# qmoututu11/Image_Restoration_and_Enhancement

Hardware: AMD Instinct MI355X
Metric: restored images/sec @512x512, 50 DDIM steps; PSNR/SSIM vs reference (higher is better)
Workload: dtype bf16; 1 GPU; BASELINE configs[1] denoise 512x512, batch 8/GPU, 50 DDIM steps x strength 0.5 = 25 UNet evals, CFG 5.0 (UNet batch 16); task=denoise, global_batch=8, resolution=512, compute=UNet + CLIP bf16, VAE fp16 (fp32 accumulation), parallelism=dp1, weights_bcast=none, outputs_finite=True

## Files before the change

image_restoration_and_enhancement_amd/_lib.py:

```python
from __future__ import annotations

import ctypes as C
import os
from pathlib import Path

_PKG = Path(__file__).resolve().parent
LIB_PATH = Path(os.environ.get("IRX_LIB", _PKG / "libirx.so"))

IRX_F32, IRX_BF16, IRX_F16 = 0, 1, 2
IRX_MODEL_UNET, IRX_MODEL_VAE, IRX_MODEL_CLIP = 0, 1, 2
IRX_MODEL_LPIPS = 3
IRX_MODEL_FID = 4
IRX_MODEL_SRVGG = 5
IRX_LAYOUT_VEC, IRX_LAYOUT_MAT, IRX_LAYOUT_CONV, IRX_LAYOUT_EMB = 0, 1, 2, 3
IRX_LAYOUT_MAT_GEGLU64, IRX_LAYOUT_VEC_GEGLU64 = 4, 5
IRX_LAYOUT_VEC_LN_U, IRX_LAYOUT_VEC_LN_V = 6, 7
IRX_LAYOUT_MAT_CHAIN, IRX_LAYOUT_VEC_CHAIN = 8, 9
IRX_LAYOUT_CONV_UP2 = 10
IRX_RCCL_ID_BYTES = 128
IRX_RESAMPLE_LANCZOS, IRX_RESAMPLE_BICUBIC, IRX_RESAMPLE_MAX_KSIZE = 0, 1, 97


class IrxError(RuntimeError):
    pass
# ... 139 lines not shown
    "irx_op_gn_proj": (i32, [vp, i32, vp, i32, i32, i32, i32, f32, vp, vp, vp, vp, i32, vp, vp, C.POINTER(i32),
                             C.POINTER(i32)]),
    "irx_op_layer_norm": (i32, [vp, i32, vp, i32, i32, f32, vp, vp, vp]),
    "irx_op_attention": (i32, [vp, i32, i32, i32, i32, i32, i32, vp, i64, i64, vp, i64, i64, vp, i64, i64, vp,
                               i64, i64, f32, i32]),
    "irx_op_attention_hm": (i32, [vp, i32, i32, i32, i32, i32, i32, vp, vp, vp, vp, f32]),
    "irx_op_geglu": (i32, [vp, i32, vp, i32, i32, vp]),
    "irx_op_gemm_geglu": (i32, [vp, i32, i32, i32, i32, vp, vp, vp, vp]),
    "irx_op_gemm_ln_out": (i32, [vp, i32, i32, i32, i32, vp, vp, vp, vp, vp, vp, i32, f32]),
    "irx_op_gemm_ln_fold": (i32, [vp, i32, i32, i32, i32, vp, vp, vp, vp, vp, vp, i32, i32, vp]),
    "irx_op_gemm_ln_out_w": (i32, [vp, i32, i32, i32, i32, vp, vp, vp, vp, i64, vp, vp, i32, i32, f32]),
    "irx_op_gemm_ln_fold_w": (i32, [vp, i32, i32, i32, i32, vp, vp, vp, vp, vp, vp, i32, i32, i32, vp]),
    "irx_op_conv2d_gn_parts": (i32, [vp, i32, vp, vp, i32, i32, i32, i32, i32, i32, i32, vp, vp, i32, i32, i32, i32,
                                     i32, i32, i32, i32, vp, i64, vp, vp, i32, i32, vp, vp, C.POINTER(i32),
                                     C.POINTER(i32), C.POINTER(i32), C.POINTER(sz)]),
    "irx_op_gemm_gn_parts": (i32, [vp, i32, i32, i32, i32, vp, vp, vp, vp, i32, vp, vp, vp, C.POINTER(i32),
                                   C.POINTER(i32), C.POINTER(sz)]),
    "irx_op_upsample_conv_gn_parts": (i32, [vp, i32, vp, i32, i32, i32, i32, vp, vp, vp, vp, vp, C.POINTER(i32),
                                            C.POINTER(i32), C.POINTER(sz)]),
    "irx_op_group_norm_parts": (i32, [vp, i32, vp, vp, i32, i32, i32, i32, i32, f32, vp, vp, i32, vp, vp, i32, vp, i32,
                                      vp]),
    "irx_op_group_norm_parts_ab": (i32, [vp, i32, i32, i32, i32, f32, vp, vp, vp, i32, vp, vp]),
    "irx_op_softmax_rows": (i32, [vp, i32, vp, i64, i32, i32, vp, i64]),
    "irx_op_transpose2d": (i32, [vp, i32, vp, i64, i32, i32, vp, i64, i32, i64, i64]),
    "irx_op_timestep_embed": (i32, [vp, i32, vp, i32, i32, i32, f32, vp]),
    "irx_op_embed_tokens": (i32, [vp, i32, vp, i32, i32, vp, vp, i32, vp]),
}

EXPORTED = tuple(_SIGS)

_DEBUG_SIGS = {
    "irx_debug_gemm_tile": (i32, [i32, i32, i32, i32, i32, i32, C.POINTER(i32)]),
    "irx_debug_conv_plan": (i32, [i32] * 17 + [C.POINTER(i32)]),
}
_SIGS.update(_DEBUG_SIGS)

_lib = None


def load(path: Path | str | None = None, force: bool = False):
    global _lib
    if _lib is not None and not force:
        return _lib
    p = Path(path) if path else LIB_PATH
    if not p.exists():
        raise IrxError(f"native library not built: {p} (run `python -m image_restoration_and_enhancement_amd.build`)")
    lib = C.CDLL(str(p))
    for name, (res, args) in _SIGS.items():
        fn = getattr(lib, name)
        fn.restype = res
        fn.argtypes = args
    _lib = lib
    return lib


def call(name: str, *args):
    lib = load()
    rc = getattr(lib, name)(*args)
    if _SIGS[name][0] is i32 and name not in ("irx_version", "irx_rccl_available") and rc != 0:
        raise IrxError(f"{name}: {lib.irx_last_error().decode(errors='replace')}")
    return rc


def get_option(name: str) -> int:
    v = C.c_int()
    call("irx_get_option", name.encode(), C.byref(v))
# ... 50 lines not shown
```

image_restoration_and_enhancement_amd/csrc/capi.cpp:

```cpp
#include <algorithm>
#include <cmath>
#include <cstring>
#include <string>

#include "../../include/irx.h"
#include "gemm_plan.h"
#include "models.h"
#include "profile.h"

namespace irx {
static thread_local std::string g_err;
void set_error(const std::string& m) { g_err = m; }
const char* last_error() { return g_err.c_str(); }
extern int g_attn_pf80;
}

using namespace irx;

struct irx_model {
  std::unique_ptr<Model> m;
};

#define IRX_API_BEGIN try {
#define IRX_API_END                                       \
// ... 31 lines not shown

const char* irx_last_error(void) { return last_error(); }
int irx_version(void) { return 1; }

struct OptRef {
  int* i = nullptr;
  bool* b = nullptr;
};
static const struct { const char* name; int* i; bool* b; } kOpts[] = {
    {"large_tiles", nullptr, &g_large_tiles},
    {"gemm_deep", &g_gemm_deep, nullptr},
    {"gemm_dbg", &g_gemm_dbg, nullptr},
    {"gn_v2", nullptr, &g_gn_v2},
    {"gn_fuse", &g_gn_fuse, nullptr},
    {"gn_parts", &g_gn_parts, nullptr},
    {"gn_red_parts", &g_gn_red_parts, nullptr},
    {"ff_chain", &g_ff_chain, nullptr},
    {"up2", &g_up2, nullptr},
    {"ln_parts", &g_ln_parts, nullptr},
    {"gn_fold", &g_gn_fold, nullptr},
    {"gn_narrow", &g_gn_narrow, nullptr},
    {"attn_pf", &g_attn_pf, nullptr},
    {"attn_pf160", &g_attn_pf160, nullptr},
    {"attn_pf80", &g_attn_pf80, nullptr},
    {"attn_q2", &g_attn_q2, nullptr},
    {"conv1x1_dense", &g_conv1x1_dense, nullptr},
    {"gn_fa", &g_gn_fa, nullptr},
    {"gn_fa_wide", &g_gn_fa_wide, nullptr},
    {"gn_fa_blocks", &g_gn_fa_blocks, nullptr},
    {"halo_split", &g_halo_split, nullptr},
    {"halo_pipe", &g_halo_pipe, nullptr},
    {"gemm_pp", &g_gemm_pp, nullptr},
    {"gemm_pp2", &g_gemm_pp2, nullptr},
    {"ln_fold", &g_ln_fold, nullptr},
    {"gemm_sk", &g_gemm_sk, nullptr},
    {"large_mask", &g_large_mask, nullptr},
    {"large_dense", &g_large_dense, nullptr},
    {"arena_guard", &g_arena_guard, nullptr},
    {"gemm_nmajor", &g_gemm_nmajor, nullptr},
    {"halo_group", &g_halo_group, nullptr},
    {"halo_strip", &g_halo_strip, nullptr},
    {"halo_up2", &g_halo_up2, nullptr},
    {"halo_mi", &g_halo_mi, nullptr},
    {"gemm_group", &g_gemm_group, nullptr},
    {"small_splitk", &g_small_splitk, nullptr},
    {"gemm_pp_chain", &g_gemm_pp_chain, nullptr},
    {"prof_shapes", &g_prof_shapes, nullptr},
    {"attn_prio", &g_attn_prio, nullptr},
    {"attn_qrep", &g_attn_qrep, nullptr},
    {"op_imgs", &g_op_imgs, nullptr},
    {"cfg_share", &g_cfg_share, nullptr},
    {"temb_table", &g_temb_table, nullptr},
    {"gemm_sk_blocks", &g_gemm_sk_blocks, nullptr},
    {"vae_attn_rows", &g_vae_attn_rows, nullptr},
    {"vae_flash", &g_vae_flash, nullptr},
    {"splitk_inkernel", nullptr, &g_splitk_inkernel},
    {"tile_256x320", nullptr, &g_tile_256x320},
    {"gemm_force", &g_gemm_force, nullptr},
    {"conv_halo", &g_conv_halo, nullptr},
    {"gemm_small", nullptr, &g_gemm_small},
    {"attn_xcd", &g_attn_xcd, nullptr},
    {"attn_hm", &g_attn_hm, nullptr},
    {"gemm_small_kmax", &g_gemm_small_kmax, nullptr},
    {"nlm2_strip", &g_nlm2_strip, nullptr},
    {"srvgg_fused", &g_srvgg_fused, nullptr},
    {"srvgg_blocks", &g_srvgg_blocks, nullptr},
// ... 682 lines not shown
  IRX_API_END
}

size_t irx_op_gemm_workspace_bytes(int dtype, int M, int N, int K, int act, int out_f32, int imgs) {
  GemmArgs a;
  a.dtype = dtype; a.M = M; a.N = N; a.K = K;
  a.A = (const void*)(uintptr_t)4096; a.lda = K;
  a.B = (const void*)(uintptr_t)4096; a.ldb = K;
  a.C = (void*)(uintptr_t)4096; a.ldc = N;
  a.act = act; a.out_f32 = out_f32; a.imgs = imgs;
  return gemm_workspace_bytes(a);
}

int irx_debug_gemm_tile(int dtype, int M, int N, int K, int geglu, int imgs, int* tile) {
  IRX_API_BEGIN
  IRX_CHECK(tile, "null argument");
  GemmArgs a;
  a.dtype = dtype; a.M = M; a.N = N; a.K = K;
  a.A = (const void*)(uintptr_t)4096; a.lda = K;
  a.B = (const void*)(uintptr_t)4096; a.ldb = K;
  a.C = (void*)(uintptr_t)4096; a.ldc = geglu ? N / 2 : N;
  a.geglu = geglu ? 1 : 0;
  a.imgs = imgs;
  const GemmPlan p = gemm_plan(a);
  const bool lt = p.path == GEMM_LARGE;
  tile[0] = lt ? p.BM : 0;
  tile[1] = lt ? p.BN : 0;
  tile[2] = lt && p.PP;
  tile[3] = !lt ? 0 : (p.PP && p.BM * p.BN == 256 * 128) || p.WM * p.WN == 4 ? 2 : 1;
  tile[4] = lt ? p.group_m : 0;
  IRX_API_END
}

int irx_debug_conv_plan(int dtype, int c0, int c1, int n, int hin, int win, int hv, int wv, int cout, int kh, int kw,
                        int stride, int pad_t, int pad_l, int ho, int wo, int out_f32, int* plan) {
  IRX_API_BEGIN
  IRX_CHECK(plan, "null argument");
  GemmArgs a;
  a.dtype = dtype;
  a.conv = 1;
  a.g.src0 = (const void*)(uintptr_t)4096;
  a.g.src1 = c1 ? (const void*)(uintptr_t)4096 : nullptr;
  a.g.C0 = c0; a.g.C1 = c1;
  a.g.N = n; a.g.Hin = hin; a.g.Win = win; a.g.Hv = hv; a.g.Wv = wv;
  a.g.KH = kh; a.g.KW = kw; a.g.stride = stride; a.g.pad_t = pad_t; a.g.pad_l = pad_l; a.g.Ho = ho; a.g.Wo = wo;
  a.M = n * ho * wo; a.N = cout; a.K = kh * kw * (c0 + c1);
  a.B = (const void*)(uintptr_t)4096; a.ldb = a.K;
  a.C = (void*)(uintptr_t)4096; a.ldc = cout; a.out_f32 = out_f32;
  a.rows_per_group = ho * wo;
  a.ldr = cout;
  a.imgs = n;
  conv1x1_as_dense(a);
  const GemmPlan p = gemm_plan(a);
  plan[0] = p.path;
  plan[1] = p.large() ? p.BM : 0;
  plan[2] = p.large() ? p.BN : 0;
  plan[3] = p.large() ? p.group_m : 0;
  plan[4] = p.large() ? p.splits : 1;
  plan[5] = p.large() ? (a.M + p.BM - 1) / p.BM : 0;
  plan[6] = p.large() ? (a.N + p.BN - 1) / p.BN : 0;
  IRX_API_END
}

int irx_op_group_norm(void* s, int dtype, const void* x0, const void* x1, int c0, int c1, int n, int hw, int groups,
                      float eps, const float* gamma, const float* beta, int silu, void* out, void* ws) {
  IRX_API_BEGIN
// ... 380 lines not shown
```

image_restoration_and_enhancement_amd/csrc/gemm2.hip:

```cpp
#include <cmath>
#include <map>
#include <mutex>
#include <type_traits>
#include <utility>

#include "gemm_plan.h"
#include "profile.h"

namespace irx {

__device__ uint4 g_zero_page[4];
#if defined(IRX_DIAG) || defined(IRX_HALO_STAMPS)
constexpr int kDbgMask = ~0;
#define IRX_HALO_DIAG 1
#else
constexpr int kDbgMask = 0;
#endif
#ifdef IRX_HALO_STAMPS
constexpr int kHaloStampBlocks = 2048;
__device__ unsigned long long g_halo_stamps[kHaloStampBlocks * 8 * 8];
extern "C" int irx_debug_halo_stamps(void* out, int n) {
  if (n > kHaloStampBlocks * 64) n = kHaloStampBlocks * 64;
  return hipMemcpyFromSymbol(out, HIP_SYMBOL(g_halo_stamps), (size_t)n * 8, 0, hipMemcpyDeviceToHost) == hipSuccess ? n : -1;
}
// ... 14 lines not shown
  unsigned* cnt = nullptr;
};

template <typename F, int... I>
__device__ __forceinline__ void static_for(std::integer_sequence<int, I...>, F&& f) {
  (f(std::integral_constant<int, I>{}), ...);
}

__device__ __forceinline__ void wait_vm(int n) {
  switch (n) {
#define IRX_VM(k) case k: asm volatile("s_waitcnt vmcnt(" #k ")" ::: "memory"); break;
    IRX_VM(0) IRX_VM(1) IRX_VM(2) IRX_VM(3) IRX_VM(4) IRX_VM(5) IRX_VM(6) IRX_VM(7) IRX_VM(8) IRX_VM(9)
    IRX_VM(10) IRX_VM(11) IRX_VM(12) IRX_VM(13) IRX_VM(14) IRX_VM(15) IRX_VM(16) IRX_VM(18) IRX_VM(20)
    IRX_VM(21) IRX_VM(24) IRX_VM(28) IRX_VM(30) IRX_VM(32) IRX_VM(35) IRX_VM(36) IRX_VM(40) IRX_VM(42)
    IRX_VM(45) IRX_VM(48) IRX_VM(49) IRX_VM(54) IRX_VM(56) IRX_VM(60)
#undef IRX_VM
    default: asm volatile("s_waitcnt vmcnt(0)" ::: "memory"); break;
  }
}

__device__ __forceinline__ void glds16_asm(const void* g, uint32_t lds_addr) {
  asm volatile("s_mov_b32 m0, %1\n\ts_nop 0\n\tglobal_load_lds_dwordx4 %0, off" ::"v"(g), "s"(lds_addr)
               : "memory", "m0");
}

__device__ __forceinline__ void glds16_s(uint32_t voff, const void* base, uint32_t lds_addr) {
  asm volatile("s_mov_b32 m0, %2\n\ts_nop 0\n\tglobal_load_lds_dwordx4 %0, %1" ::"v"(voff), "s"(base), "s"(lds_addr)
               : "memory", "m0");
}

constexpr int kStripEdgeL = 320, kStripEdgeR = 336;
static_assert(kStripEdgeR + 16 <= 256 + 2 * kHaloWMax, "strip halo edge columns");

constexpr bool pp_pair(bool pp, int bm, int bn) { return pp && bm * bn == 256 * 128; }

template <typename T, int BM, int BN, int WM, int WN, int BK, int S, bool CONV, bool OUTF32, bool RESIZE,
          int HALO = 0, bool PP = false>
__global__ __launch_bounds__(WM * WN * 64, pp_pair(PP, BM, BN) ? 4 : WM * WN == 4 ? 2 : 1) void gemm2_kernel(GemmArgs a,
                                                                                                            Split sp) {
  constexpr int NW = WM * WN, NT = NW * 64;
  constexpr bool PAIR = pp_pair(PP, BM, BN);
  if constexpr (PAIR) {
    a.A1 = nullptr; a.b_rows = 0; a.rowadd = nullptr; a.gn_part = nullptr; a.ln_out = nullptr; a.up2_w = 0;
    sp.splits = 1;
  }
  constexpr int TM = BM / WM / 16, TN = BN / WN / 16;
  constexpr int ROWS = BM + BN;
  constexpr int CPR = BK / 8;
  constexpr int RPI = 64 / CPR;
  constexpr int NINST = ROWS / RPI;
  constexpr int IPW = (NINST + NW - 1) / NW;
  constexpr int STAGE = ROWS * CPR;
  constexpr int KSUB = BK / 32;
  static_assert((NW == 8 || NW == 4) && ROWS % RPI == 0 && BM % 16 == 0 && (BK == 32 || BK == 64), "tile shape");
  static_assert(!HALO || (CONV && !RESIZE && S >= 2 && S <= 8 && NW == 8), "halo tiles: 3x3 conv");
  static_assert(!PP || !CONV, "ping-pong: dense GEMMs only");
  constexpr bool STRIP = HALO == 5 || HALO == 7;
  constexpr int NTAP = (HALO == 6 || HALO == 7 || HALO == 9) ? 4 : 9;
  constexpr bool MI = HALO == 8 || HALO == 9;
  constexpr int HB_U4 = (BM + 2 * kHaloWMax) * CPR;
  constexpr int RING = HALO ? 2 * HB_U4 + S * BN * CPR + CPR + 64 : S * STAGE;
  constexpr int RINGX = RING + (!HALO && NINST % NW ? 64 : 0);
  constexpr int SMEM = RINGX > BM * BN / 8 ? RINGX : BM * BN / 8;
  static_assert(SMEM * 16 <= 160 * 1024, "LDS budget");
  constexpr bool LNTAB = !CONV && !OUTF32 && HALO == 0 && SMEM * 16 + BM * 8 <= 160 * 1024;
  constexpr int LNT_U4 = LNTAB ? BM / 2 : 0;
  static_assert(!LNTAB || NT >= BM, "one thread per table row");
// ... 541 lines not shown
#pragma unroll
        for (int ss = 0; ss < KSUB; ++ss) {
          const int ck = ss * 4 + fgrp;
#pragma unroll
          for (int i = 0; i < TM; ++i) {
            const int r = wm * TM * 16 + i * 16 + frow;
            const int rx = r & (W - 1);
            const int hp = r + shift;
            const bool zero = (kx == 0 && rx == 0) || (kx == 2 && rx == W - 1);
            af[ss][i] = zero ? zrow[ck] : Hs[hp * CPR + (ck ^ swz(hp))];
          }
#pragma unroll
          for (int j = 0; j < TN; ++j) {
            const int r = wn * TN * 16 + j * 16 + frow;
            bfr[ss][j] = Bs[r * CPR + (ck ^ swz(r))];
          }
        }
        __builtin_amdgcn_s_setprio(1);
#pragma unroll
        for (int ss = 0; ss < KSUB; ++ss)
#pragma unroll
          for (int i = 0; i < TM; ++i)
#pragma unroll
            for (int j = 0; j < TN; ++j)
              acc[i][j] = Mfma<T>::m16x16x32(af[ss][i], bfr[ss][j], acc[i][j]);
        __builtin_amdgcn_s_setprio(0);
      }
      if (gab && t >= S && 9 * (c + 1) < nk) transformH(c + 1, t - S, t - S + 1);
      st = st + 1 == S ? 0 : st + 1;
    }
    asm volatile("s_waitcnt vmcnt(0)" ::: "memory");
    __syncthreads();
  } else if constexpr (PP) {
    static_assert(S == 3 && NW == 8, "ping-pong: 3 stages, 8 waves");
    const int wv = __builtin_amdgcn_readfirstlane(wave);
    const bool g1 = wv >= NW / 2;
    const uint32_t lds0 = __builtin_amdgcn_readfirstlane((uint32_t)(uintptr_t)(lds_void*)smem);
    const char* pb[IPW];
    const char* pb1[IPW];
    uint32_t pv[IPW], pv1[IPW], pd[IPW];
    bool apc[IPW];
#pragma unroll
    for (int j = 0; j < IPW; ++j) {
      const int q = wv * IPW + j, r0 = RPI * q, r = r0 + lrow;
      const int ch = (lslot ^ swz(r)) * 8;
      apc[j] = q < NINST && r0 < BM;
      if (q < NINST && r0 < BM) {
        pb[j] = (const char*)(Ap + (long)(m0 + r0) * a.lda);
        pv[j] = (uint32_t)(lrow * a.lda + ch) * 2u;
      } else if (q < NINST) {
        pb[j] = (const char*)(Bp + (long)(n0 + r0 - BM) * a.ldb);
        pv[j] = (uint32_t)(lrow * a.ldb + ch) * 2u;
      } else {
        pb[j] = (const char*)(Ap + (long)m0 * a.lda);
        pv[j] = (uint32_t)lane * 16u;
      }
      pd[j] = q < NINST ? lds0 + (uint32_t)(q * 64) * 16u : lds0 + (uint32_t)(SMEM - 64) * 16u;
      pb1[j] = pb[j];
      pv1[j] = pv[j];
      if (A1p && apc[j]) {
        pb1[j] = (const char*)(A1p + (long)(m0 + r0) * a.lda1);
        pv1[j] = (uint32_t)(lrow * a.lda1 + ch) * 2u;
      }
    }
    auto issueP = [&](int kt, int st) {
      const long ko = (long)kt * BK * 2;
      const bool second = A1p && kt * BK >= a.kA1;
// ... 10 lines not shown
    auto readF = [&](auto stc) {
      constexpr int st = decltype(stc)::value;
      const uint4* As = smem + st * STAGE;
      const uint4* Bs = As + BM * CPR;
#pragma unroll
      for (int s = 0; s < KSUB; ++s) {
#pragma unroll
        for (int i = 0; i < TM; ++i) {
          const int r = wm * TM * 16 + i * 16 + frow;
          fa[s][i] = As[r * CPR + ((s * 4 + fgrp) ^ swz(r))];
        }
#pragma unroll
        for (int j = 0; j < TN; ++j) {
          const int r = wn * TN * 16 + j * 16 + frow;
          fb[s][j] = Bs[r * CPR + ((s * 4 + fgrp) ^ swz(r + BM))];
        }
      }
    };
    auto mma = [&]() {
#pragma unroll
      for (int s = 0; s < KSUB; ++s)
#pragma unroll
        for (int i = 0; i < TM; ++i)
#pragma unroll
          for (int j = 0; j < TN; ++j) acc[i][j] = Mfma<T>::m16x16x32(fa[s][i], fb[s][j], acc[i][j]);
    };
    auto barrier = [&](bool drain) {
      __builtin_amdgcn_sched_barrier(0);
      if (drain) asm volatile("s_waitcnt lgkmcnt(0)\n\ts_barrier" ::: "memory");
      else asm volatile("s_barrier" ::: "memory");
      __builtin_amdgcn_sched_barrier(0);
    };
    issueP(kt0, 0);
    issueP(min(kt0 + 1, kt1 - 1), 1);
    ln_table();
    wait_vm(IPW);
    barrier(true);
    if (g1) barrier(true);
    for (int kb = kt0; kb < kt1; kb += 3) {
      static_for(std::make_integer_sequence<int, 3>{}, [&](auto uc) {
        constexpr int u = decltype(uc)::value;
        const int kt = kb + u;
        if (kt < kt1) {
          readF(uc);
          issueP(min(kt + 2, kt1 - 1), (u + 2) % 3);
          if (g1) wait_vm(IPW);
          barrier(g1);
          mma();
          if (!g1) wait_vm(IPW);
          barrier(true);
        }
      });
    }
    if (!g1) barrier(true);
    asm volatile("s_waitcnt vmcnt(0)" ::: "memory");
    __syncthreads();
  } else if constexpr (S == 2) {
    if (kt0 < kt1) issue(kt0, 0);
    ln_table();
    asm volatile("s_waitcnt vmcnt(0)" ::: "memory");
    __syncthreads();
    for (int kt = kt0; kt < kt1; ++kt) {
      const int st = (kt - kt0) & 1;
      if (kt + 1 < kt1) issue(kt + 1, st ^ 1);
      if (!(a.dbg & kDbgMask & 2)) compute(st);
      asm volatile("s_waitcnt vmcnt(0)" ::: "memory");
      __syncthreads();
    }
  } else {
#pragma unroll
    for (int p = 0; p < S - 1; ++p)
      if (kt0 + p < kt1) issue(kt0 + p, p);
    ln_table();
    int st = 0;
    for (int kt = kt0; kt < kt1; ++kt) {
      wait_vm(IPW * min(S - 2, kt1 - 1 - kt));
      asm volatile("s_barrier" ::: "memory");
      if (kt + S - 1 < kt1) issue(kt + S - 1, st == 0 ? S - 1 : st - 1);
      if (!(a.dbg & kDbgMask & 2)) compute(st);
      st = st + 1 == S ? 0 : st + 1;
    }
    asm volatile("s_waitcnt vmcnt(0)" ::: "memory");
// ... 631 lines not shown
  sp.splits = p.splits;
  sp.per = p.per;
  if (p.splits > 1) {
    sp.Mp = p.Mp;
    sp.Np = p.Np;
    sp.ws = (a.splitk_ws && a.splitk_ws_bytes >= p.ws_bytes) ? (float*)a.splitk_ws : internal_ws(p.ws_bytes);
    sp.inkernel = p.inkernel;
    if (sp.inkernel) sp.cnt = stream_counters(s);
  }
#ifdef IRX_HALO_DIAG
  if (p.path == GEMM_HALO && g_halo_pipe && !a.gn_ab && b.dbg && a.dtype == BF16) {
    launch2<256, 160, 4, 2, 64, 3, 4>(b, sp, s);
    return;
  }
#endif
#define IRX_K2(...) case gemm2_key(__VA_ARGS__): launch2<__VA_ARGS__>(b, sp, s); break;
  switch (gemm2_key(p.BM, p.BN, p.WM, p.WN, p.BK, p.S, p.HALO, p.PP)) {
    IRX_K2(256, 160, 4, 2, 64, 3, 9, false)
    IRX_K2(256, 160, 4, 2, 64, 3, 8, false)
    IRX_K2(256, 128, 4, 2, 64, 3, 7, false)
    IRX_K2(256, 160, 4, 2, 64, 3, 6, false)
    IRX_K2(256, 128, 4, 2, 64, 3, 6, false)
    IRX_K2(256, 160, 4, 2, 64, 3, 5, false)
    IRX_K2(256, 128, 4, 2, 64, 3, 5, false)
    IRX_K2(256, 160, 4, 2, 64, 3, 2, false)
    IRX_K2(256, 128, 4, 2, 64, 3, 2, false)
    IRX_K2(256, 160, 4, 2, 64, 3, 1, false)
    IRX_K2(64, 320, 1, 4, 32, 2, 0, false)
    IRX_K2(128, 160, 2, 2, 64, 2, 0, false)
    IRX_K2(128, 128, 2, 2, 64, 2, 0, false)
    IRX_K2(256, 320, 2, 4, 32, 3, 0, true)
    IRX_K2(256, 256, 2, 4, 32, 3, 0, true)
    IRX_K2(128, 320, 2, 4, 32, 3, 0, true)
    IRX_K2(256, 128, 4, 2, 32, 3, 0, true)
    IRX_K2(128, 256, 2, 4, 32, 3, 0, true)
    IRX_K2(256, 128, 4, 2, 64, 3, 0, false)
    IRX_K2(128, 256, 2, 4, 64, 3, 0, false)
    IRX_K2(128, 128, 2, 4, 64, 4, 0, false)
    IRX_K2(256, 160, 4, 2, 64, 3, 0, false)
    IRX_K2(256, 256, 2, 4, 32, 4, 0, false)
    IRX_K2(128, 320, 2, 4, 32, 5, 0, false)
    IRX_K2(256, 128, 4, 2, 32, 5, 0, false)
    IRX_K2(128, 256, 2, 4, 32, 5, 0, false)
    IRX_K2(128, 128, 2, 4, 32, 6, 0, false)
    IRX_K2(256, 320, 2, 4, 64, 2, 0, false)
    IRX_K2(256, 256, 2, 4, 64, 2, 0, false)
    IRX_K2(128, 320, 2, 4, 64, 2, 0, false)
    IRX_K2(256, 128, 4, 2, 64, 2, 0, false)
    IRX_K2(128, 256, 2, 4, 64, 2, 0, false)
    IRX_K2(128, 128, 2, 4, 64, 2, 0, false)
    default: IRX_CHECK(false, "gemm_large_tile: the plan names a kernel that is not instantiated");
  }
#undef IRX_K2
}

}
```

image_restoration_and_enhancement_amd/csrc/gemm_plan.cpp:

```cpp
#include "gemm_plan.h"

#include <algorithm>
#include <cmath>

namespace irx {

bool g_large_tiles = true;
int g_large_mask = 3;
int g_large_dense = 63;
int g_small_splitk = 1;
int g_gemm_sk = 1;
int g_gemm_deep = 0;
bool g_gemm_small = false;
int g_gemm_small_kmax = 1280;
int g_gemm_force = 0;
bool g_tile_256x320 = true;
bool g_splitk_inkernel = true;
int g_gemm_nmajor = 1;
int g_gemm_group = 1;
int g_gemm_pp = 2;
int g_gemm_pp2 = 1;
int g_gemm_pp_chain = 1;
int g_conv1x1_dense = 1;
int g_conv_halo = 1;
int g_halo_split = 1;
int g_halo_pipe = 1;
int g_halo_strip = 1;
int g_halo_up2 = 1;
int g_halo_mi = 1;
int g_halo_group = 1;
int g_gn_fuse = 0;
int g_gn_parts = 1;
int g_gn_red_parts = 1;
int g_gn_fold = 1;
int g_ln_fold = 1;
int g_ln_parts = 1;

namespace {

constexpr int kCUs = 256;
constexpr long kPairMinTiles = 2L * kCUs;

struct Choice {
  int BM = 0, BN = 0, splits = 1, per = 0;
  bool small = false;
  bool pair = false;
};

int step_k() { return g_gemm_deep == 1 ? 32 : 64; }

long canon_rows(const GemmArgs& a) {
  const long rows = (long)a.M * a.batch;
  return a.imgs > 0 ? rows / a.imgs * kCanonImages : rows;
}
// ... 51 lines not shown
    }
  }
  return best;
}

bool vec_ok(const GemmArgs& a) {
  return !a.out_f32 && a.N % 8 == 0 && a.ldc % 8 == 0 && ((uintptr_t)a.C % 16) == 0 &&
         (!a.residual || (a.ldr % 8 == 0 && ((uintptr_t)a.residual % 16) == 0)) &&
         (a.batch == 1 || (a.sC % 8 == 0 && (!a.residual || a.sR % 8 == 0)));
}

bool pair_form(const GemmArgs& a) {
  return g_gemm_pp2 && g_gemm_pp && g_gemm_deep == 0 && !g_gemm_small && g_gemm_force == 0 && !a.conv && !a.A1 &&
         !a.b_rows && !a.rowadd && !a.gn_part && !a.gn_ab && !a.ln_out && !a.up2_w && a.K % 32 == 0;
}

bool pair_tile(const GemmArgs& a, const Choice& c, int& BM, int& BN) {
  if (!pair_form(a)) return false;
  int bm = 256, bn = 128;
  if (g_gemm_pp2 >= 2) {
    if (g_gemm_pp2 == 3) { bm = 128; bn = 256; }
  } else {
    if (c.splits != 1 || a.K % 64 != 0) return false;
    const long tiles = canon_rows(a) / bm * (a.N / bn);
    const bool geglu = a.geglu && c.BM == 256 && c.BN == 256 && tiles >= kCUs;
    const bool wide = !a.geglu && c.BM == 128 && c.BN == 320 && a.K >= 640 && tiles >= kPairMinTiles;
    if (!geglu && !wide) return false;
  }
  if (a.M % bm != 0 || a.N % bn != 0) return false;
  BM = bm; BN = bn;
  return true;
}

bool eligible(const GemmArgs& a) {
  const int bk = (g_gemm_pp2 >= 2 && pair_form(a)) ? 32 : step_k();
  if (!(g_large_mask & (a.conv ? 2 : 1))) return false;
  if (!a.conv && g_large_dense != 63) {
    const int cls = a.geglu ? (a.K <= 320 ? 4 : a.K <= 640 ? 16 : 32) : a.hs_L ? 2 : a.N <= 1280 ? 1 : 8;
    if (!(g_large_dense & cls)) return false;
  }
  if (a.hs_L && !vec_ok(a)) return false;
  if (a.act != ACT_NONE) return false;
  if (!vec_ok(a) && (a.rowadd || a.residual)) return false;
  if (a.rowadd && (a.rowadd_ld % 4 != 0 || ((uintptr_t)a.rowadd % 16) != 0)) return false;
  if (!is16(a.dtype) || a.K % bk != 0 || a.ldb % 8 != 0) return false;
  if (canon_rows(a) < 512) return false;
  if (a.geglu && (a.out_f32 || a.residual || a.batch != 1 || a.N % 128 != 0)) return false;
  if (a.conv) return !a.out_f32 && a.g.C0 % bk == 0 && a.g.C1 % bk == 0;
  if (a.A1 && (a.batch != 1 || a.kA1 % 64 != 0 || a.lda1 % 8 != 0 || ((uintptr_t)a.A1 % 16) != 0)) return false;
  return a.lda % 8 == 0 && (a.batch == 1 || a.sA % 8 == 0);
}

int small_splits(const GemmArgs& a) {
  if (!g_small_splitk || !is16(a.dtype) || a.conv || a.batch != 1 || a.geglu || a.A1 || a.up2_w) return 0;
  if (a.M > 256 || a.N % 8 || a.K < 1024 || a.N <= 16) return 0;
  if (a.out_f32 ? a.ldc % 4 != 0 : (a.ldc % 8 != 0 || ((uintptr_t)a.C % 16) != 0)) return 0;
  if (a.residual && (a.ldr % 8 != 0 || ((uintptr_t)a.residual % 16) != 0)) return 0;
  const long ctiles = (a.N + 63) / 64;
  if (ctiles >= 128) return 0;
  int sp = 1;
  while (sp < 8 && ctiles * sp * 2 <= 256 && a.K % (sp * 2 * 64) == 0 && a.K / (sp * 2) >= 256) sp *= 2;
  return sp > 1 ? sp : 0;
}

struct Halo {
  int mode = 0;
  int bn = 0;
  int splits = 1;
// ... 89 lines not shown

void plan_halo_launch(const GemmArgs& a, const Halo& h, GemmPlan& p) {
  p.path = GEMM_HALO;
  p.vec_epilogue = true;
  p.group_m = halo_group_m(a, h);
  const bool mi = h.mode == 3;
  int halo;
  if (mi) halo = a.up2_w ? 9 : 8;
  else if (a.up2_w) halo = h.mode == 2 ? 7 : 6;
  else if (h.mode == 2) halo = 5;
  else halo = g_halo_pipe && !a.gn_ab ? 2 : 1;
  set_kernel(p, 256, h.bn, 4, 2, 64, 3, halo);
  p.splits = h.splits;
  p.per = a.K / 64;
  if (h.splits > 1) {
    const int slabs = (a.g.C0 + a.g.C1) / 64;
    p.per = (a.up2_w ? 4 : 9) * ((slabs + h.splits - 1) / h.splits);
    p.Mp = (a.M + 255) / 256 * 256;
    p.Np = a.N;
    p.ws_bytes = (size_t)h.splits * p.Mp * a.N * sizeof(float);
    p.inkernel = !mi;
  }
}

bool large_kernel(const GemmArgs& a, const Choice& c, GemmPlan& p) {
  const int key = c.BM * 1000 + c.BN;
  const int wm = (c.BM == 256 && c.BN <= 160) ? 4 : 2, wn = 8 / wm;
  if (c.pair) {
    set_kernel(p, c.BM, c.BN, wm, wn, 32, 3, 0, true);
  } else if (c.BM == 64) {
    set_kernel(p, 64, 320, 1, 4, 32, 2);
  } else if (c.small) {
    set_kernel(p, 128, c.BN, 2, 2, 64, 2);
  } else if (g_gemm_deep == 0 && g_gemm_pp && !a.conv && !a.ln_out && !a.b_rows &&
             (!a.A1 || g_gemm_pp_chain) &&
             ((c.BM == 256 && c.BN == 256) ||
              (a.A1 && g_gemm_pp_chain && c.BN == 320 && (c.BM == 256 || c.BM == 128) && a.K >= 1024)) &&
             a.M % c.BM == 0 && a.N % c.BN == 0) {
    set_kernel(p, c.BM, c.BN, wm, wn, 32, 3, 0, true);
  } else if (g_gemm_deep == 2) {
    if (key == 256320) return false;
    set_kernel(p, c.BM, c.BN, wm, wn, 64, (key == 256256 || key == 128320) ? 2 : key == 128128 ? 4 : 3);
  } else if (g_gemm_deep == 1) {
    if (key == 256320 || c.BN == 160) return false;
    set_kernel(p, c.BM, c.BN, wm, wn, 32, key == 256256 ? 4 : key == 128128 ? 6 : 5);
  } else {
    if (c.BN == 160) return false;
    set_kernel(p, c.BM, c.BN, wm, wn, 64, 2);
  }
  return true;
}

bool plan_large(const GemmArgs& a, const Choice& c0, GemmPlan& p) {
  Choice c = c0;
  if (pair_tile(a, c0, c.BM, c.BN)) {
    c.pair = true;
    c.splits = 1;
  } else if (a.K % step_k() != 0) {
    return false;
  }
  const bool vec = vec_ok(a);
  if (a.geglu && !vec) return false;
  if (c.splits > 1) {
    if (!vec && !a.out_f32) return false;
    if (a.out_f32 && (a.ldc % 8 != 0 || a.N % 8 != 0)) return false;
  }
  if (!large_kernel(a, c, p)) return false;
  p.path = GEMM_LARGE;
  p.vec_epilogue = vec;
  p.nmajor = g_gemm_nmajor == 2 || (g_gemm_nmajor == 1 && (long)a.N * a.batch > (long)a.M * a.batch);
  if (a.batch == 1 && !a.hs_L) {
    p.group_m = dense_group_m(a, c.BM, c.BN, (c.BM == 128 && c.BN == 128) || c.small || c.pair ? 2 : 1, p.nmajor);
    if (p.group_m) p.nmajor = 0;
  }
  p.splits = c.splits;
  p.per = c.pair ? a.K / p.BK : (c.splits > 1 ? c.per : a.K / step_k()) * (step_k() / p.BK);
  if (c.splits > 1) {
    p.Mp = (a.M + c.BM - 1) / c.BM * c.BM;
    p.Np = (a.N + c.BN - 1) / c.BN * c.BN;
    p.ws_bytes = (size_t)c.splits * a.batch * p.Mp * p.Np * sizeof(float);
    p.inkernel = reduce_in_kernel(c.splits, (long)(p.Mp / c.BM) * (p.Np / c.BN) * a.batch);
  }
  return true;
}

template <typename T> T* requested() { return (T*)(uintptr_t)4096; }

}

bool gemm_sk_eligible(const GemmArgs& a) {
  if (!g_gemm_sk || (!a.geglu && g_gemm_sk != 3) || !is16(a.dtype) || a.conv || a.out_f32 || a.batch != 1 || a.K != kSkK) return false;
  if (a.act != ACT_NONE || a.rowadd || a.gn_part || a.gn_ab || a.b_rows || a.ln_out) return false;
  if (a.A1 || a.up2_w) return false;
  if (a.res_rows) return false;
  if (a.geglu ? (a.N % 256 != 0 || a.N / 2 / 128 > 32 || a.residual || a.hs_L || a.ldc % 4) : (a.N % 320 || a.N / 320 > 32))
    return false;
  if (a.lda % 8 || a.ldb % 8 || ((uintptr_t)a.A % 16) || ((uintptr_t)a.B % 16)) return false;
  if (((uintptr_t)a.C % 8) || (a.hs_L ? (a.hs_d % 4 || a.hs_C % 4) : a.ldc % 4)) return false;
  if (a.residual && (a.ldr % 4 || ((uintptr_t)a.residual % 8))) return false;
  if (a.hs_L && (a.residual || a.hs_L % 64)) return false;
  if ((a.ln_rs || a.ln_part) && (a.alpha != 1.f || a.M % 2)) return false;
  if (a.ln_part && a.ln_T != 1) return false;
  return a.M > 0;
}

GemmPlan gemm_plan(const GemmArgs& a) {
  GemmPlan p;
  const int small = small_splits(a);
  const size_t small_bytes = small ? (size_t)small * a.M * a.N * sizeof(float) : 0;
// ... 116 lines not shown
```

image_restoration_and_enhancement_amd/csrc/ops.h:

```cpp
#pragma once
#include "irx_common.h"

namespace irx {

struct ConvGeom {
  const void* src0 = nullptr;
  const void* src1 = nullptr;
  int C0 = 0, C1 = 0;
  int N = 0, Hin = 0, Win = 0;
  int Hv = 0, Wv = 0;
  int KH = 1, KW = 1, stride = 1, pad_t = 0, pad_l = 0;
  int Ho = 0, Wo = 0;
};

struct GemmArgs {
  int dtype = BF16;
  int M = 0, N = 0, K = 0;
  int conv = 0;
  ConvGeom g;
  const void* A = nullptr; long lda = 0; long sA = 0;
  const void* A1 = nullptr; long lda1 = 0; int kA1 = 0;
  const void* B = nullptr; long ldb = 0; long sB = 0;
  void* C = nullptr; long ldc = 0; long sC = 0;
  int out_f32 = 0;
// ... 65 lines not shown
}
#define c_off(a, m, n) c_off_f((m), (n), (a).ldc, (a).M, (a).hs_L, (a).hs_C, (a).hs_d, (a).up2_w, (a).up2_p)
void gemm(const GemmArgs& a, hipStream_t s);
bool gemm_sk(const GemmArgs& a, hipStream_t s);
bool gemm_sk_eligible(const GemmArgs& a);
float* splitk_scratch(size_t bytes);
void splitk_reduce(const GemmArgs& a, const float* ws, int splits, int Mp, int Np, int batch, hipStream_t s);
bool conv1x1_as_dense(GemmArgs& a);
size_t gemm_workspace_bytes(const GemmArgs& a);
size_t gemm_small_split_bytes(const GemmArgs& a);
int gemm_large_splits(const GemmArgs& a);
bool gemm_up2_ok(const GemmArgs& a);
bool gemm_geglu_fusable(const GemmArgs& a);
bool gemm_gn_fusable(const GemmArgs& a);
bool gemm_ln_foldable(const GemmArgs& a);
bool gemm_emits_ln_parts(const GemmArgs& a);
bool gemm_bimg_ok(const GemmArgs& a);
int gemm_emits_gn_parts(const GemmArgs& a);
extern bool g_large_tiles;
extern int g_large_mask;
extern int g_large_dense;
extern int g_small_splitk;
extern int g_gemm_sk;
extern int g_gemm_deep;
extern bool g_gemm_small;
extern int g_gemm_small_kmax;
extern int g_gemm_force;
extern bool g_tile_256x320;
extern bool g_splitk_inkernel;
extern int g_gemm_nmajor;
extern int g_gemm_group;
extern int g_gemm_pp;
extern int g_gemm_pp2;
extern int g_gemm_pp_chain;
extern int g_conv1x1_dense;
extern int g_conv_halo;
extern int g_halo_split;
extern int g_halo_pipe;
extern int g_halo_strip;
extern int g_halo_up2;
extern int g_halo_mi;
extern int g_halo_group;
extern int g_gn_fuse;
extern int g_gn_parts;
extern int g_gn_red_parts;
extern int g_gn_fold;
extern int g_ln_fold;
extern int g_ln_parts;
extern int g_gemm_sk_blocks;
extern int g_gemm_dbg;
extern int g_up2;
extern int g_ff_chain;

size_t gn_ws_bytes(int N, int HW, int G);
extern int g_gn_fa;
extern int g_gn_fa_wide;
extern int g_gn_fa_blocks;
extern bool g_gn_v2;
void group_norm(int dtype, const void* x0, const void* x1, int C0, int C1, int N, int HW, int G, float eps,
                const float* gamma, const float* beta, int silu, void* out, void* ws, hipStream_t s);
void group_norm_parts(int dtype, const void* x0, const void* x1, int C0, int C1, int N, int HW, int G, float eps,
                      const float* gamma, const float* beta, int silu, void* out, const double* p0, int r0,
                      const double* p1, int r1, void* ws, hipStream_t s);
void group_norm_stats(int dtype, const void* x0, const void* x1, int C0, int C1, int N, int HW, int G, float eps,
                      const float* gamma, const float* beta, float2* ab, void* ws, hipStream_t s);
void group_norm_parts_ab(int C0, int N, int HW, int G, float eps, const float* gamma, const float* beta,
// ... 139 lines not shown
```

Measured before the change: 18.18 images/s.

## Generalize ping-pong GEMM to deeper LDS rings and add 128x128 ring tile

Generalizes the ping-pong GEMM mainloop from a fixed three-stage LDS ring to a templated depth of 3 to 5 stages, with more loads in flight and counted vmcnt waits scaled to match. With the default ring setting, plain GEMMs that fit in one wave of 128x128 tiles (no split-K, K a multiple of 64, long enough K loop) now use a new 4-stage ping-pong 128x128 kernel. A forced mode switches other ping-pong tiles to deeper rings. The trade-off is more LDS per block, which can lower occupancy, in exchange for hiding more global-load latency on small-grid GEMMs. A debug API reports the chosen ring depth.

```diff
diff --git a/image_restoration_and_enhancement_amd/_lib.py b/image_restoration_and_enhancement_amd/_lib.py
--- a/image_restoration_and_enhancement_amd/_lib.py
+++ b/image_restoration_and_enhancement_amd/_lib.py
@@ -195,6 +195,7 @@
 _DEBUG_SIGS = {
     "irx_debug_gemm_tile": (i32, [i32, i32, i32, i32, i32, i32, C.POINTER(i32)]),
     "irx_debug_conv_plan": (i32, [i32] * 17 + [C.POINTER(i32)]),
+    "irx_debug_gemm_ring": (i32, [i32] * 7 + [C.POINTER(i32)]),
 }
 _SIGS.update(_DEBUG_SIGS)
 
diff --git a/image_restoration_and_enhancement_amd/csrc/capi.cpp b/image_restoration_and_enhancement_amd/csrc/capi.cpp
--- a/image_restoration_and_enhancement_amd/csrc/capi.cpp
+++ b/image_restoration_and_enhancement_amd/csrc/capi.cpp
@@ -87,6 +87,7 @@
     {"halo_pipe", &g_halo_pipe, nullptr},
     {"gemm_pp", &g_gemm_pp, nullptr},
     {"gemm_pp2", &g_gemm_pp2, nullptr},
+    {"gemm_ring", &g_gemm_ring, nullptr},
     {"ln_fold", &g_ln_fold, nullptr},
     {"gemm_sk", &g_gemm_sk, nullptr},
     {"large_mask", &g_large_mask, nullptr},
@@ -835,6 +836,30 @@
   IRX_API_END
 }
 
+int irx_debug_gemm_ring(int dtype, int M, int N, int K, int kA1, int feat, int imgs, int* ring) {
+  IRX_API_BEGIN
+  IRX_CHECK(ring, "null argument");
+  GemmArgs a;
+  a.dtype = dtype; a.M = M; a.N = N; a.K = K;
+  a.A = (const void*)(uintptr_t)4096; a.lda = kA1 > 0 ? kA1 : K;
+  if (kA1 > 0) { a.A1 = (const void*)(uintptr_t)4096; a.lda1 = K - kA1; a.kA1 = kA1; }
+  a.B = (const void*)(uintptr_t)4096; a.ldb = K;
+  a.C = (void*)(uintptr_t)4096; a.ldc = N;
+  if (feat & 1) { a.residual = (const void*)(uintptr_t)4096; a.ldr = N; }
+  if (feat & 2) a.ln_rs = (const float2*)(uintptr_t)4096;
+  if (feat & 4) a.gn_part = (double*)(uintptr_t)4096;
+  if (feat & 8) { a.ln_out = (float2*)(uintptr_t)4096; a.ln_W = N >= kLnGroup && N % kLnGroup == 0 ? kLnGroup : kLnGroupNarrow; }
+  a.imgs = imgs;
+  const GemmPlan p = gemm_plan(a);
+  const bool lt = p.path == GEMM_LARGE;
+  ring[0] = lt ? p.BM : 0;
+  ring[1] = lt ? p.BN : 0;
+  ring[2] = lt && p.PP;
+  ring[3] = lt ? p.S : 0;
+  ring[4] = lt ? p.splits : 0;
+  IRX_API_END
+}
+
 int irx_debug_conv_plan(int dtype, int c0, int c1, int n, int hin, int win, int hv, int wv, int cout, int kh, int kw,
                         int stride, int pad_t, int pad_l, int ho, int wo, int out_f32, int* plan) {
   IRX_API_BEGIN
diff --git a/image_restoration_and_enhancement_amd/csrc/gemm2.hip b/image_restoration_and_enhancement_amd/csrc/gemm2.hip
--- a/image_restoration_and_enhancement_amd/csrc/gemm2.hip
+++ b/image_restoration_and_enhancement_amd/csrc/gemm2.hip
@@ -70,7 +70,7 @@
 constexpr int kStripEdgeL = 320, kStripEdgeR = 336;
 static_assert(kStripEdgeR + 16 <= 256 + 2 * kHaloWMax, "strip halo edge columns");
 
-constexpr bool pp_pair(bool pp, int bm, int bn) { return pp && bm * bn == 256 * 128; }
+constexpr bool pp_pair(bool pp, int bm, int bn) { return pp && (bm * bn == 256 * 128 || bm * bn == 128 * 128); }
 
 template <typename T, int BM, int BN, int WM, int WN, int BK, int S, bool CONV, bool OUTF32, bool RESIZE,
           int HALO = 0, bool PP = false>
@@ -678,7 +678,10 @@
     asm volatile("s_waitcnt vmcnt(0)" ::: "memory");
     __syncthreads();
   } else if constexpr (PP) {
-    static_assert(S == 3 && NW == 8, "ping-pong: 3 stages, 8 waves");
+    static_assert(S >= 3 && S <= 5 && NW == 8, "ping-pong: 3 to 5 stages, 8 waves");
+    static_assert(S == 3 || SMEM * 16 + (LNTAB ? BM * 8 : 0) <= 160 * 1024, "ping-pong ring + LayerNorm table in LDS");
+    static_assert(S == 3 || !pp_pair(PP, BM, BN) || 2 * (SMEM * 16 + BM * 8) <= 160 * 1024, "two resident blocks");
+    static_assert(IPW * (S - 2) <= 16, "counted wait inside wait_vm's table");
     const int wv = __builtin_amdgcn_readfirstlane(wave);
     const bool g1 = wv >= NW / 2;
     const uint32_t lds0 = __builtin_amdgcn_readfirstlane((uint32_t)(uintptr_t)(lds_void*)smem);
@@ -755,22 +758,25 @@
       __builtin_amdgcn_sched_barrier(0);
     };
     issueP(kt0, 0);
-    issueP(min(kt0 + 1, kt1 - 1), 1);
+    static_for(std::make_integer_sequence<int, S - 2>{}, [&](auto pc) {
+      constexpr int p = decltype(pc)::value + 1;
+      issueP(min(kt0 + p, kt1 - 1), p);
+    });
     ln_table();
-    wait_vm(IPW);
+    wait_vm(IPW * (S - 2));
     barrier(true);
     if (g1) barrier(true);
-    for (int kb = kt0; kb < kt1; kb += 3) {
-      static_for(std::make_integer_sequence<int, 3>{}, [&](auto uc) {
+    for (int kb = kt0; kb < kt1; kb += S) {
+      static_for(std::make_integer_sequence<int, S>{}, [&](auto uc) {
         constexpr int u = decltype(uc)::value;
         const int kt = kb + u;
         if (kt < kt1) {
           readF(uc);
-          issueP(min(kt + 2, kt1 - 1), (u + 2) % 3);
-          if (g1) wait_vm(IPW);
+          issueP(min(kt + S - 1, kt1 - 1), (u + S - 1) % S);
+          if (g1) wait_vm(IPW * (S - 2));
           barrier(g1);
           mma();
-          if (!g1) wait_vm(IPW);
+          if (!g1) wait_vm(IPW * (S - 2));
           barrier(true);
         }
       });
@@ -1468,6 +1474,10 @@
     IRX_K2(256, 320, 2, 4, 32, 3, 0, true)
     IRX_K2(256, 256, 2, 4, 32, 3, 0, true)
     IRX_K2(128, 320, 2, 4, 32, 3, 0, true)
+    IRX_K2(256, 320, 2, 4, 32, 4, 0, true)
+    IRX_K2(256, 256, 2, 4, 32, 4, 0, true)
+    IRX_K2(128, 320, 2, 4, 32, 5, 0, true)
+    IRX_K2(128, 128, 2, 4, 32, 4, 0, true)
     IRX_K2(256, 128, 4, 2, 32, 3, 0, true)
     IRX_K2(128, 256, 2, 4, 32, 3, 0, true)
     IRX_K2(256, 128, 4, 2, 64, 3, 0, false)
diff --git a/image_restoration_and_enhancement_amd/csrc/gemm_plan.cpp b/image_restoration_and_enhancement_amd/csrc/gemm_plan.cpp
--- a/image_restoration_and_enhancement_amd/csrc/gemm_plan.cpp
+++ b/image_restoration_and_enhancement_amd/csrc/gemm_plan.cpp
@@ -20,6 +20,7 @@
 int g_gemm_group = 1;
 int g_gemm_pp = 2;
 int g_gemm_pp2 = 1;
+int g_gemm_ring = 1;
 int g_gemm_pp_chain = 1;
 int g_conv1x1_dense = 1;
 int g_conv_halo = 1;
@@ -137,8 +138,35 @@
   return true;
 }
 
+bool ring_form(const GemmArgs& a) {
+  return g_gemm_ring && g_gemm_pp && g_gemm_deep == 0 && !g_gemm_small && !a.conv && !a.ln_out && !a.b_rows &&
+         !a.gn_ab && a.K % 32 == 0;
+}
+bool ring_forced(const GemmArgs& a) { return g_gemm_ring == 2 && ring_form(a); }
+
+int ring_max(int key) { return key == 128320 ? 5 : (key == 256256 || key == 256320 || key == 128128) ? 4 : 3; }
+
+int ring_steps(const GemmArgs& a, const Choice& c) {
+  const int nk = a.K / 32;
+  if (c.splits <= 1) return nk;
+  const int per = c.per * (step_k() / 32);
+  return std::min(per, nk - (c.splits - 1) * per);
+}
+
+int ring_depth(const GemmArgs& a, const Choice& c) {
+  return g_gemm_ring == 2 ? ring_max(c.BM * 1000 + c.BN) : 3;
+}
+
+bool ring_tile128(const GemmArgs& a, const Choice& c) {
+  if (!ring_form(a) || c.BM != 128 || c.BN != 128 || c.small || c.pair || c.splits != 1) return false;
+  if (a.A1 || a.rowadd || a.gn_part || a.up2_w || a.geglu || a.M % 128 != 0 || a.N % 128 != 0) return false;
+  if (g_gemm_ring == 2) return true;
+  const long tiles = (canon_rows(a) + 127) / 128 * (a.N / 128);
+  return g_gemm_force == 0 && tiles <= kCUs &&a.K % 64 == 0 && !a.out_f32 && a.batch == 1 && ring_steps(a, c) >= ring_max(128128) + 2;
+}
+
 bool eligible(const GemmArgs& a) {
-  const int bk = (g_gemm_pp2 >= 2 && pair_form(a)) ? 32 : step_k();
+  const int bk = ((g_gemm_pp2 >= 2 && pair_form(a)) || ring_forced(a)) ? 32 : step_k();
   if (!(g_large_mask & (a.conv ? 2 : 1))) return false;
   if (!a.conv && g_large_dense != 63) {
     const int cls = a.geglu ? (a.K <= 320 ? 4 : a.K <= 640 ? 16 : 32) : a.hs_L ? 2 : a.N <= 1280 ? 1 : 8;
@@ -294,12 +322,15 @@
     set_kernel(p, 64, 320, 1, 4, 32, 2);
   } else if (c.small) {
     set_kernel(p, 128, c.BN, 2, 2, 64, 2);
+  } else if (ring_tile128(a, c)) {
+    set_kernel(p, 128, 128, 2, 4, 32, ring_max(128128), 0, true);
   } else if (g_gemm_deep == 0 && g_gemm_pp && !a.conv && !a.ln_out && !a.b_rows &&
              (!a.A1 || g_gemm_pp_chain) &&
              ((c.BM == 256 && c.BN == 256) ||
-              (a.A1 && g_gemm_pp_chain && c.BN == 320 && (c.BM == 256 || c.BM == 128) && a.K >= 1024)) &&
+              (a.A1 && g_gemm_pp_chain && c.BN == 320 && (c.BM == 256 || c.BM == 128) && a.K >= 1024) ||
+              (ring_forced(a) && c.BN == 320 && (c.BM == 256 || c.BM == 128))) &&
              a.M % c.BM == 0 && a.N % c.BN == 0) {
-    set_kernel(p, c.BM, c.BN, wm, wn, 32, 3, 0, true);
+    set_kernel(p, c.BM, c.BN, wm, wn, 32, ring_depth(a, c), 0, true);
   } else if (g_gemm_deep == 2) {
     if (key == 256320) return false;
     set_kernel(p, c.BM, c.BN, wm, wn, 64, (key == 256256 || key == 128320) ? 2 : key == 128128 ? 4 : 3);
@@ -318,7 +349,7 @@
   if (pair_tile(a, c0, c.BM, c.BN)) {
     c.pair = true;
     c.splits = 1;
-  } else if (a.K % step_k() != 0) {
+  } else if (a.K % step_k() != 0 && !(ring_forced(a) && c.splits == 1)) {
     return false;
   }
   const bool vec = vec_ok(a);
@@ -327,7 +358,9 @@
     if (!vec && !a.out_f32) return false;
     if (a.out_f32 && (a.ldc % 8 != 0 || a.N % 8 != 0)) return false;
   }
-  if (!large_kernel(a, c, p)) return false;
+  GemmPlan k;
+  if (!large_kernel(a, c, k) || a.K % k.BK != 0) return false;
+  set_kernel(p, k.BM, k.BN, k.WM, k.WN, k.BK, k.S, k.HALO, k.PP);
   p.path = GEMM_LARGE;
   p.vec_epilogue = vec;
   p.nmajor = g_gemm_nmajor == 2 || (g_gemm_nmajor == 1 && (long)a.N * a.batch > (long)a.M * a.batch);
@@ -336,7 +369,7 @@
     if (p.group_m) p.nmajor = 0;
   }
   p.splits = c.splits;
-  p.per = c.pair ? a.K / p.BK : (c.splits > 1 ? c.per : a.K / step_k()) * (step_k() / p.BK);
+  p.per = c.pair || c.splits == 1 ? a.K / p.BK : c.per * (step_k() / p.BK);
   if (c.splits > 1) {
     p.Mp = (a.M + c.BM - 1) / c.BM * c.BM;
     p.Np = (a.N + c.BN - 1) / c.BN * c.BN;
diff --git a/image_restoration_and_enhancement_amd/csrc/ops.h b/image_restoration_and_enhancement_amd/csrc/ops.h
--- a/image_restoration_and_enhancement_amd/csrc/ops.h
+++ b/image_restoration_and_enhancement_amd/csrc/ops.h
@@ -121,6 +121,7 @@
 extern int g_gemm_group;
 extern int g_gemm_pp;
 extern int g_gemm_pp2;
+extern int g_gemm_ring;
 extern int g_gemm_pp_chain;
 extern int g_conv1x1_dense;
 extern int g_conv_halo;
```

Result: no change. 18.23 images/s (median of 6 runs) (+0.2%).
